# ntampellini/FIRECODE

Hardware: AMD Instinct MI355X
Metric: conformer-pair RMSD alignments/s (higher is better)
Workload: dtype f64

## Files before the change

firecode_amd/csrc/fc_api_ensemble.cpp:

```cpp
#include <algorithm>
#include <cmath>
#include <cstdlib>
#include <memory>

#include "fc_internal.h"

namespace fc {

static int make_selection(const uint8_t *atom_mask, int64_t A_all, std::vector<int32_t> &sel) {
  sel.clear();
  for (int64_t a = 0; a < A_all; ++a)
    if (atom_mask == nullptr || atom_mask[a]) sel.push_back((int32_t)a);
  if (sel.empty()) return set_error(FC_E_INVALID, "atom_mask selects no atom");
  return FC_OK;
}

int ensemble_build_finish(fc_ensemble *e) {
  if (!e->g_max_pending) return FC_OK;
  e->g_max_pending = false;
  FC_TRY(sync());
  std::memcpy(&e->g_max, ctx().pinned_word, sizeof(double));
  auto *gmax_dev = reinterpret_cast<unsigned long long *>(e->counters.p) + (kCounters - 1);
  FC_HIP_TRY(hipMemsetAsync(gmax_dev, 0, sizeof(unsigned long long), ctx().stream));
  return FC_OK;
// ... 283 lines not shown
  FC_REQUIRE(P >= 0, "P < 0");
  if (P == 0) return FC_OK;
  FC_REQUIRE(pair_i && pair_j && rmsd_out && maxdev_out, "NULL pointer argument");
  for (int64_t k = 0; k < P; ++k)
    FC_REQUIRE(pair_i[k] >= 0 && pair_i[k] < ens->N && pair_j[k] >= 0 && pair_j[k] < ens->N,
               "pair %lld = (%lld, %lld) out of range [0, %lld)", (long long)k,
               (long long)pair_i[k], (long long)pair_j[k], (long long)ens->N);
  FC_TRY(ensure_init());
  DevBuf di, dj, dr, dm;
  FC_TRY(upload(di, pair_i, (size_t)P));
  FC_TRY(upload(dj, pair_j, (size_t)P));
  FC_TRY(dr.reserve((size_t)P * sizeof(double)));
  FC_TRY(dm.reserve((size_t)P * sizeof(double)));
  FC_TRY(launch_pairs_exact(ens, di.as<int64_t>(), dj.as<int64_t>(), P, dr.as<double>(),
                            dm.as<double>(), nullptr, inverted));
  FC_TRY(d2h(rmsd_out, dr.p, (size_t)P * sizeof(double)));
  FC_TRY(d2h(maxdev_out, dm.p, (size_t)P * sizeof(double)));
  return sync();
}
int fc_ensemble_rmsd_pairs(fc_ensemble *ens, const int64_t *pair_i, const int64_t *pair_j,
                           int64_t P, double *rmsd_out, double *maxdev_out) {
  return ensemble_rmsd_pairs(ens, pair_i, pair_j, P, rmsd_out, maxdev_out, false);
}
int fc_ensemble_rmsd_pairs_inv(fc_ensemble *ens, const int64_t *pair_i, const int64_t *pair_j, int64_t P, double *rmsd_out,
                               double *maxdev_out) {
  return ensemble_rmsd_pairs(ens, pair_i, pair_j, P, rmsd_out, maxdev_out, true);
}

static int kabsch_rmsd_pairs(const double *coords, int64_t N, int64_t A, const uint8_t *atom_mask, const int64_t *pair_i,
                             const int64_t *pair_j, int64_t P, int center, double *rmsd_out, double *maxdev_out,
                             bool inverted) {
  FC_API_LOCK;
  fc_ensemble *e = nullptr;
  FC_TRY(fc_ensemble_create(coords, N, A, atom_mask, center, &e));
  const int rc = ensemble_rmsd_pairs(e, pair_i, pair_j, P, rmsd_out, maxdev_out, inverted);
  fc_ensemble_destroy(e);
  return rc;
}
int fc_kabsch_rmsd_pairs(const double *coords, int64_t N, int64_t A, const uint8_t *atom_mask,
                         const int64_t *pair_i, const int64_t *pair_j, int64_t P, int center,
                         double *rmsd_out, double *maxdev_out) {
  return kabsch_rmsd_pairs(coords, N, A, atom_mask, pair_i, pair_j, P, center, rmsd_out, maxdev_out, false);
}
int fc_kabsch_rmsd_pairs_inv(const double *coords, int64_t N, int64_t A, const uint8_t *atom_mask, const int64_t *pair_i,
                             const int64_t *pair_j, int64_t P, int center, double *rmsd_out, double *maxdev_out) {
  return kabsch_rmsd_pairs(coords, N, A, atom_mask, pair_i, pair_j, P, center, rmsd_out, maxdev_out, true);
}

static bool rmsd_and_max_tiled(const fc_ensemble *ens) {
  const size_t lds_m = ((size_t)(((ens->A + 3) / 4 + 1) / 2) * 384 + 16 + 128) * sizeof(double) + 1024;
  return lds_m <= kLdsLimit && (uint64_t)((ens->A + 3) / 4 * 4) * 3 * (uint64_t)ens->Npad < (1ull << 32);
}

static int rmsd_and_max_all(fc_ensemble *ens, double *rmsd_out, double *maxdev_out, double *ms_kernel) {
  FC_TRY(ensure_init());
  const int64_t N = ens->N;
  if (N == 0) return FC_OK;
  Context &c = ctx();
  DevBuf dr, dm;
  const size_t bytes = (size_t)N * N * sizeof(double);
  FC_TRY(dr.reserve(bytes));
  FC_TRY(dm.reserve(bytes));
  const bool tiled = rmsd_and_max_tiled(ens);
  unsigned long long cnt[16] = {0};
  if (tiled) {
    FC_TRY(ensemble_shard(ens, 0, 1, 256));
    FC_HIP_TRY(hipMemsetAsync(ens->counters.p, 0, 16 * sizeof(uint64_t), c.stream));
  } else {
    FC_HIP_TRY(hipMemsetAsync(dr.p, 0, bytes, c.stream));
    FC_HIP_TRY(hipMemsetAsync(dm.p, 0, bytes, c.stream));
  }
  FC_HIP_TRY(hipEventRecord(c.ev0, c.stream));
  if (tiled) FC_TRY(launch_rmsd_values(ens, 0.0, dr.as<double>(), dm.as<double>()));
  else FC_TRY(launch_matrix_exact(ens, dr.as<double>(), dm.as<double>()));
  FC_HIP_TRY(hipEventRecord(c.ev1, c.stream));
  if (tiled) FC_TRY(d2h(cnt, ens->counters.p, sizeof cnt));
  FC_TRY(sync());
  FC_TRY(elapsed_ms(c.ev0, c.ev1, ms_kernel));
  if (tiled && cnt[6] > (unsigned long long)ens->pairq_cap) {
    FC_HIP_TRY(hipMemsetAsync(ens->counters.p, 0, 16 * sizeof(uint64_t), c.stream));
    FC_TRY(launch_rmsd_values(ens, 0.0, dr.as<double>(), dm.as<double>(), 0, 1, true));
    FC_TRY(d2h(cnt, ens->counters.p, sizeof cnt));
    FC_TRY(sync());
  }
  if (tiled && cnt[6] > (unsigned long long)ens->pairq_cap) {
    FC_HIP_TRY(hipMemsetAsync(dr.p, 0, bytes, c.stream));
    FC_HIP_TRY(hipMemsetAsync(dm.p, 0, bytes, c.stream));
    FC_TRY(launch_matrix_exact(ens, dr.as<double>(), dm.as<double>()));
  }
  if (rmsd_out) FC_TRY(launch_mirror_upper(dr.as<double>(), N));
  if (maxdev_out) FC_TRY(launch_mirror_upper(dm.as<double>(), N));
  if (rmsd_out) FC_TRY(d2h(rmsd_out, dr.p, bytes));
  if (maxdev_out) FC_TRY(d2h(maxdev_out, dm.p, bytes));
  return sync();
}

static int bench_rmsd_and_max_all(fc_ensemble *ens, int64_t reps, double *ms_kernel_mean, double *ms_total,
                                  int64_t *stats, const int64_t *sample_i = nullptr, const int64_t *sample_j = nullptr,
                                  int64_t P = 0, double *sample_rmsd = nullptr, double *sample_maxdev = nullptr) {
  FC_TRY(ensure_init());
  const int64_t N = ens->N;
  FC_REQUIRE(N >= 2, "needs at least two conformers");
  Context &c = ctx();
  DevBuf dr, dm;
  const size_t bytes = (size_t)N * N * sizeof(double);
  FC_TRY(dr.reserve(bytes));
  FC_TRY(dm.reserve(bytes));
  const bool tiled = rmsd_and_max_tiled(ens);
  const int64_t rank = comm_rank(), world = comm_world();
  FC_REQUIRE(tiled || world == 1, "structures beyond the tiled kernel are not sharded");
  if (tiled) FC_TRY(ensemble_shard(ens, 0, 1, 256));
  FC_TRY(timing_events(2 * reps + 2));
  std::vector<hipEvent_t> &ev = c.ev_pool;
  FC_HIP_TRY(hipEventRecord(ev[2 * reps], c.stream));
  for (int64_t r = 0; r < reps; ++r) {
    if (tiled) {
      FC_HIP_TRY(hipMemsetAsync(ens->counters.p, 0, 16 * sizeof(uint64_t), c.stream));
      FC_HIP_TRY(hipEventRecord(ev[2 * r], c.stream));
      c.mark_after_screen = ev[2 * r + 1];
      const int rc = launch_rmsd_values(ens, 0.0, dr.as<double>(), dm.as<double>(), rank, world);
      c.mark_after_screen = nullptr;
      FC_TRY(rc);
    } else {
      FC_HIP_TRY(hipEventRecord(ev[2 * r], c.stream));
      FC_TRY(launch_matrix_exact(ens, dr.as<double>(), dm.as<double>()));
      FC_HIP_TRY(hipEventRecord(ev[2 * r + 1], c.stream));
    }
  }
  FC_HIP_TRY(hipEventRecord(ev[2 * reps + 1], c.stream));
  unsigned long long cnt[16] = {0};
  if (tiled) FC_TRY(d2h(cnt, ens->counters.p, sizeof cnt));
  FC_TRY(sync());
  double mean = 0.0;
  FC_TRY(mean_elapsed_ms(ev, reps, 2, 1, &mean));
  if (ms_kernel_mean) *ms_kernel_mean = mean;
  FC_TRY(elapsed_ms(ev[2 * reps], ev[2 * reps + 1], ms_total));
  if (stats) {
    stats[0] = owned_pairs(N, 128, rank, world);
    stats[1] = (int64_t)cnt[6];
    stats[2] = tiled ? 1 : 0;
    stats[3] = (int64_t)cnt[kCntGeneralForm];
  }
  if (tiled && cnt[6] > (unsigned long long)ens->pairq_cap)
    return set_error(FC_E_LIMIT, "%llu degenerate pairs exceed the fix-up queue (%lld)", cnt[6], (long long)ens->pairq_cap);
  if (P > 0) {
    DevBuf di, dj, sr, sm;
    FC_TRY(upload(di, sample_i, (size_t)P));
    FC_TRY(upload(dj, sample_j, (size_t)P));
    FC_TRY(sr.reserve((size_t)P * sizeof(double)));
    FC_TRY(sm.reserve((size_t)P * sizeof(double)));
    FC_TRY(launch_gather_matrix_pairs(dr.as<double>(), dm.as<double>(), N, di.as<int64_t>(), dj.as<int64_t>(), P,
                                      sr.as<double>(), sm.as<double>()));
    FC_TRY(d2h(sample_rmsd, sr.p, (size_t)P * sizeof(double)));
    FC_TRY(d2h(sample_maxdev, sm.p, (size_t)P * sizeof(double)));
    FC_TRY(sync());
  }
  return FC_OK;
}

int fc_ensemble_rmsd_matrix(fc_ensemble *ens, double *rmsd_out, double *maxdev_out) {
  FC_API_LOCK;
  FC_REQUIRE(ens && rmsd_out && maxdev_out, "NULL pointer argument");
  return rmsd_and_max_all(ens, rmsd_out, maxdev_out, nullptr);
}
// ... 94 lines not shown
```

firecode_amd/csrc/fc_kabsch.hip:

```cpp
#include <type_traits>

#include "fc_internal.h"
#include <vector>
#include "fc_kabsch_math.h"

#include <algorithm>
#include <cstdlib>

namespace fc {

__global__ void __launch_bounds__(256)
k_prep(const double *__restrict__ coords, int64_t N, int64_t A_all, const int32_t *__restrict__ sel,
       int64_t A, int center, int64_t Npad, double *__restrict__ Xs, double *__restrict__ G,
       double *__restrict__ Xa, unsigned long long *__restrict__ gmax_bits,
       const int32_t *__restrict__ conf_idx) {
  const int64_t n = (int64_t)blockIdx.x * blockDim.x + threadIdx.x;
  if (n >= Npad) return;
  for (int64_t a = A; a < ((A + 3) & ~(int64_t)3); ++a) {
    Xs[(a * 3 + 0) * Npad + n] = 0.0;
    Xs[(a * 3 + 1) * Npad + n] = 0.0;
    Xs[(a * 3 + 2) * Npad + n] = 0.0;
  }
  if (n >= N) {
    for (int64_t a = 0; a < A; ++a) {
// ... 617 lines not shown
  if (i0 >= N) return;
  if (j0 + TC - 1 <= i0) return;
  uint32_t *__restrict__ sq32_wave = reinterpret_cast<uint32_t *>(stageQ) + wv * (kStagePairs * 2 / NW);
  int n_staged32 = 0;
  (void)sq32_wave;
  (void)n_staged32;

  {
    const int n_runs = TC == 64 ? KS * 6 : (TC == 32 ? KS * 3 : ((KS + 1) >> 1) * 3);
    const int cs_l = TC == 64 ? lane >> 4 : lane >> 5, k1_l = TC == 64 ? (lane >> 3) & 1 : (lane >> 3) & 3, c15_l = (lane & 7) * 2;
    for (int q = wv; q < n_runs; q += NW) {
      const int sc = TC == 64 ? q >> 1 : q, kh = TC == 64 ? q & 1 : 0;
      const int sg = sc / 3, c = sc - sg * 3;
      int a = sg * 4 + kh * 2 + k1_l;
      if (TC == 16) {
        a = (sg * 2 + cs_l) * 4 + k1_l;
        a = a < KS * 4 ? a : KS * 4 - 1;
      }
      const double *src = Xs + (int64_t)(a * 3 + c) * Npad + j0 + (TC == 16 ? 0 : cs_l * 16) + c15_l;
      __builtin_amdgcn_global_load_lds((const __attribute__((address_space(1))) void *)src,
                                       (__attribute__((address_space(3))) void *)(lds + q * 128), 16, 0, 0);
    }
    for (int idx = tid; idx < TC + IB; idx += NW * 64) {
      const int64_t g = idx < TC ? j0 + idx : i0 + (idx - TC);
      ldsG[idx] = g < Npad ? G[g] : 0.0;
    }
    if (tid < kStagePairs) stageQ[tid] = ~0ull;
    if (tid < kStageWords) stageW[tid] = ~0u;
    if (tid < 2) stageN[tid] = 0u;
    __syncthreads();
#ifdef FC_TIMELINE
    if (TL && tl && tid == 0) tl[(size_t)b * 4 + 1] = wall_clock64();
#endif
  }
  const int kq = lane >> 4, l15 = lane & 15;
  const int lcol = MODE == 2 ? 4 * (l15 & 3) + (l15 >> 2) : l15;
  const int boff = (kq / KPR) * 128 + (kq % KPR) * 16 + lcol;
  uint16_t *bits16 = reinterpret_cast<uint16_t *>(bits);

  double a0[3], a1[3], a2[3];
  int pre_it = -1;
  int n_general = 0;
  (void)n_general;
  (void)general_only;
  const int tpb = IB >> 4;
  auto tile_row = [&](int it_) -> int64_t {
    if constexpr (MODE == 2) {
      const int k = it_ / tpb;
      return global_block(lb + k, rank, world) * IB + (int64_t)(it_ - k * tpb) * 16;
    } else {
      return i0 + (int64_t)it_ * 16;
    }
  };
  auto row_offsets = [&](int it_, unsigned (&vo)[3]) {
    const int64_t ib_ = tile_row(it_);
#pragma unroll
    for (int c = 0; c < 3; ++c) vo[c] = (unsigned)(((int64_t)(kq * 3 + c) * Npad + ib_ + l15) * 8);
  };
  auto fetch_a_at = [&](double (&a)[3], unsigned (&vo)[3], int sx) {
    const int sl = sx < KS ? sx : KS - 1;
    const char *__restrict__ xs_s = reinterpret_cast<const char *>(Xs + (int64_t)sl * 12 * Npad);
#pragma unroll
    for (int c = 0; c < 3; ++c) {
      asm volatile("" : "+v"(vo[c]));
      a[c] = *reinterpret_cast<const double *>(xs_s + vo[c]);
    }
  };

  for (int it = it_first + wv; it < it_last; it += NW) {
    const int64_t ib = tile_row(it);
    if (ib >= N) break;
    if (j0 + TC - 1 <= ib) break;
    const int64_t lrow0 = lb * IB + (int64_t)it * 16;
    double Gp_row = 0.0;
    if constexpr (MODE == 2) Gp_row = G[ib + l15];
    (void)Gp_row;
    unsigned nz = 0;
    unsigned voff[3];
    row_offsets(it, voff);

#pragma unroll 1
    for (int half = 0; half < NU; ++half) {
      const int cs0 = half * NT;
      if (j0 + (cs0 + NT) * 16 - 1 <= ib) {
        if (!VALUES && lane < 16 && ib + lane < N) {
          bits16[((lrow0 + lane) * W + jt) * 4 + cs0] = 0;
          bits16[((lrow0 + lane) * W + jt) * 4 + cs0 + 1] = 0;
        }
        continue;
      }
      if constexpr (MODE == 2) {
        if (j0 + cs0 * 16 >= N) continue;
      }
      d4_t acc[NT][9];

      const double *__restrict__ lb0 = lds + cs0 * SST + boff;
      double b0[NT][3], b1[NT][3];
      const int KSe = KS;
      auto fetch_a = [&](double (&a)[3], int sx) {
        fetch_a_at(a, voff, sx);
      };
      auto fetch_b = [&](double (&b)[NT][3], int sx) {
        const int sl = sx < KS ? sx : KS - 1;
        const double *__restrict__ lb_s = lb0 + koff(sl);
#pragma unroll
        for (int t = 0; t < NT; ++t)
#pragma unroll
          for (int c = 0; c < 3; ++c) b[t][c] = lb_s[c * CST + t * SST];
      };
      auto mma = [&](const double (&a)[3], const double (&b)[NT][3], auto first_) {
        constexpr bool first = decltype(first_)::value;
#pragma unroll
        for (int x = 0; x < 3; ++x)
#pragma unroll
          for (int y = 0; y < 3; ++y)
#pragma unroll
            for (int t = 0; t < NT; ++t) {
              const d4_t c_in = first ? d4_t{0.0, 0.0, 0.0, 0.0} : acc[t][x * 3 + y];
              acc[t][x * 3 + y] = MODE == 2 ? __builtin_amdgcn_mfma_f64_16x16x4f64(b[t][y], a[x], c_in, 0, 0, 0)
                                            : __builtin_amdgcn_mfma_f64_16x16x4f64(a[x], b[t][y], c_in, 0, 0, 0);
            }
      };
      if (pre_it != it) {
        fetch_a_at(a0, voff, 0);
        fetch_a_at(a1, voff, 1);
        fetch_a_at(a2, voff, 2);
      }
      fetch_b(b0, 0);
      fetch_b(b1, 1);
#define FC_KSTEP(AX, BX, U)             \
  if (sgrp + (U) < KSe) {               \
    mma(AX, BX, std::false_type{});     \
    fetch_a(AX, sgrp + (U) + 3);        \
    fetch_b(BX, sgrp + (U) + 2);        \
  }
      mma(a0, b0, std::true_type{});
      fetch_a(a0, 3);
      fetch_b(b0, 2);
      for (int sgrp = 1; sgrp < KSe; sgrp += 6) {
        FC_KSTEP(a1, b1, 0)
        FC_KSTEP(a2, b0, 1)
        FC_KSTEP(a0, b1, 2)
        FC_KSTEP(a1, b0, 3)
        FC_KSTEP(a2, b1, 4)
        FC_KSTEP(a0, b0, 5)
      }
#undef FC_KSTEP
      {
        const bool same_tile = half < NU - 1 && !(MODE == 2 && j0 + (cs0 + NT) * 16 >= N);
        const int nit = same_tile ? it : it + NW;
        bool more = same_tile;
        if (!same_tile && nit < it_last) {
          const int64_t nib = tile_row(nit);
          more = nib < N && !(j0 + TC - 1 <= nib);
        }
        if (more) {
          unsigned vn[3];
          row_offsets(nit, vn);
          fetch_a_at(a0, vn, 0);
          fetch_a_at(a1, vn, 1);
          fetch_a_at(a2, vn, 2);
          pre_it = nit;
        } else {
          pre_it = -1;
        }
      }
      const int n32 = (int)N, ib32 = (int)ib;
#pragma unroll
      for (int t = 0; t < NT; ++t) {
        const int cs = cs0 + t;
        const int j = (int)j0 + cs * 16 + l15;
        const double Gq = ldsG[cs * 16 + l15];
        uint64_t mr[4] = {0, 0, 0, 0};
        if (MODE == 2) {
          const int i = ib32 + l15;
          const int jb = (int)j0 + cs * 16 + 4 * kq;
          const double Gp = Gp_row;
          double nR[4][9];
          bool ok4[4];
          double msdA4[4] = {0.0, 0.0, 0.0, 0.0};
          {
            if constexpr (COL0) {
              double B4[4][9], GG[4], lam4[4];
#pragma unroll
              for (int r = 0; r < 4; ++r) {
                GG[r] = Gp + ldsG[cs * 16 + 4 * kq + r];
#pragma unroll
                for (int e = 0; e < 9; ++e) B4[r][e] = acc[t][e][r];
              }
              QcpLeanPoly P4[4];
              double dl4[4];
              qcp_lean_eigenvalues4(B4, GG, P4, lam4, dl4);
              bool conv4[4];
#pragma unroll
              for (int r = 0; r < 4; ++r) conv4[r] = qcp_lean_converged(lam4[r], dl4[r]);
              bool all_lean = true, try_col0 = general_only == 0;
              const double k_small = 2e-10 / (double)A;
#pragma unroll
              for (int r = 0; r < 4; ++r) {
                double Qr[4], nqr;
                bool lean = false;
                if (try_col0) {
                  ok4[r] = qcp_lean_quaternion_col0(B4[r], P4[r].n2, lam4[r], conv4[r], Qr, nqr);
                  lean = __builtin_amdgcn_ballot_w64(!(ok4[r] || i >= n32 || jb + r >= n32)) == 0ull;
                  try_col0 = lean;
                }
                if (!lean) ok4[r] = qcp_lean_quaternion_raw(B4[r], P4[r].n2, lam4[r], conv4[r], Qr, nqr);
                all_lean = all_lean && lean;
                if constexpr (EIG) {
                  msdA4[r] = GG[r] - 2.0 * lam4[r];
                  if (!(msdA4[r] > k_small * GG[r] * GG[r])) ok4[r] = false, msdA4[r] = 0.0;
                }
                if (!lean && !ok4[r]) Qr[0] = 1.0, Qr[1] = 0.0, Qr[2] = 0.0, Qr[3] = 0.0, nqr = 1.0;
                neg_rotation_from_raw_quaternion(Qr, nqr, nR[r]);
              }
              if (!all_lean) ++n_general;
            } else {
              double B4[4][9], GG[4], Q44[4][4], nq4[4], lam4[4];
#pragma unroll
              for (int r = 0; r < 4; ++r) {
                GG[r] = Gp + ldsG[cs * 16 + 4 * kq + r];
#pragma unroll
                for (int e = 0; e < 9; ++e) B4[r][e] = acc[t][e][r];
              }
              kabsch_quaternion_qcp_lean4(B4, GG, Q44, nq4, ok4, EIG ? lam4 : nullptr);
              ++n_general;
              if constexpr (EIG) {
                const double k_small = 2e-10 / (double)A;
#pragma unroll
                for (int r = 0; r < 4; ++r) {
                  msdA4[r] = GG[r] - 2.0 * lam4[r];
                  if (!(msdA4[r] > k_small * GG[r] * GG[r])) ok4[r] = false, msdA4[r] = 0.0;
                }
              }
#pragma unroll
              for (int r = 0; r < 4; ++r) {
                if (!ok4[r]) Q44[r][0] = 1.0, Q44[r][1] = 0.0, Q44[r][2] = 0.0, Q44[r][3] = 0.0, nq4[r] = 1.0;
                neg_rotation_from_raw_quaternion(Q44[r], nq4[r], nR[r]);
              }
            }
          }
          typedef double d2_t __attribute__((ext_vector_type(2)));
          const double *__restrict__ qcol = lds + cs * SST + 4 * kq;
          const double *__restrict__ prow_u = Xs + ib;
          const unsigned l15u = (unsigned)l15;
// ... 107 lines not shown
            double PA[3], PB[3];
            load_pq(U0{}, PA, QA);
            for (int g = 0; g < n_groups; ++g) {
              load_pq(U1{}, PB, QB);
              FC_SB;
              accumulate(PA, QA);
              FC_SB;
              load_pq(U2{}, PA, QA);
              FC_SB;
              accumulate(PB, QB);
              FC_SB;
              load_pq(U3{}, PB, QB);
              FC_SB;
              accumulate(PA, QA);
              FC_SB;
              qg = TC == 16 ? qcol + koff(g + 1) : qg + 12 * TC;
              if (g + 1 < n_groups || odd_round) load_pq(U0{}, PA, QA);
              FC_SB;
              accumulate(PB, QB);
              FC_SB;
            }
            if (odd_round) {
              load_pq(U1{}, PB, QB);
              FC_SB;
              accumulate(PA, QA);
              FC_SB;
              accumulate(PB, QB);
            }
          }
#undef FC_SB
          if constexpr (EIG) {
#pragma unroll
            for (int r = 0; r < 4; ++r) ssq[r] = msdA4[r];
          }
          const bool row_in = i < n32;
          double *__restrict__ ro = rmsd_out + (int64_t)i * N + jb;
          double *__restrict__ mo = maxdev_out + (int64_t)i * N + jb;
          const double invA = 1.0 / (double)A;
          if (row_in && jb > i && jb + 3 < n32 && ((((int64_t)i * N) & 1) == 0)) {
            *reinterpret_cast<d2_t *>(ro) = d2_t{fc_sqrt_nonneg(ssq[0] * invA), fc_sqrt_nonneg(ssq[1] * invA)};
            *reinterpret_cast<d2_t *>(ro + 2) = d2_t{fc_sqrt_nonneg(ssq[2] * invA), fc_sqrt_nonneg(ssq[3] * invA)};
            *reinterpret_cast<d2_t *>(mo) = d2_t{fc_sqrt_nonneg(mx[0]), fc_sqrt_nonneg(mx[1])};
            *reinterpret_cast<d2_t *>(mo + 2) = d2_t{fc_sqrt_nonneg(mx[2]), fc_sqrt_nonneg(mx[3])};
          } else {
#pragma unroll
            for (int r = 0; r < 4; ++r) {
              const int j = jb + r;
              if (row_in && j >= i && j < n32) {
                ro[r] = j == i ? 0.0 : fc_sqrt_nonneg(ssq[r] * invA);
                mo[r] = j == i ? 0.0 : fc_sqrt_nonneg(mx[r]);
              }
            }
          }
#pragma unroll
          for (int r = 0; r < 4; ++r) {
            const int j = jb + r;
            const bool redo = row_in && (j > i) && (j < n32) && !ok4[r];
            stage_pairs(__ballot(redo), redo, (unsigned)i, (unsigned)j, stageQ, stageN, pairq, Q, counters, lane);
          }
          continue;
        }
#pragma unroll
        for (int r = 0; r < 4; ++r) {
          const int i = ib32 + kq + 4 * r;
          const double Gp = ldsG[TC + it * 16 + kq + 4 * r];
          double B9[9];
#pragma unroll
          for (int e = 0; e < 9; ++e) B9[e] = acc[t][e][r];
          if (VALUES) {
            double slope;
            const double lam = kabsch_lambda_max(B9, Gp + Gq, &slope);
            const double msdA = (Gp + Gq) - 2.0 * lam;
            const bool in = (j > i) && (j < n32) && (i < n32);
            if (in) rmsd_out[(int64_t)i * N + j] = sqrt(fmax(msdA, 0.0) / (double)A);
            const bool redo = in && (msdA < A_thr2 || !kabsch_lambda_is_sharp(lam, slope, (double)A, msdA));
            stage_pairs(__ballot(redo), redo, (unsigned)i, (unsigned)j, stageQ, stageN, pairq, Q, counters, lane);
            continue;
          }
          bool may = kabsch_may_be_below<ENANT>(B9, Gp + Gq, A_thr2);
          may = may && (j > i) && (j < n32) && (i < n32);
          mr[r] = __ballot(may);
          if constexpr (MODE == 0)
            stage_pairs_wave32<kStagePairs * 2 / NW>(mr[r], may, (unsigned)i, (unsigned)j, (unsigned)i0, (unsigned)j0, sq32_wave,
                                                     n_staged32, pairq, Q, counters, lane);
          else
            stage_pairs(mr[r], may, (unsigned)i, (unsigned)j, stageQ, stageN, pairq, Q, counters, lane);
        }
        if (!VALUES && lane < 16 && ib32 + lane < n32) {
          const int rr = lane >> 2;
          const uint64_t mine = rr == 0 ? mr[0] : rr == 1 ? mr[1] : rr == 2 ? mr[2] : mr[3];
          const unsigned piece = (unsigned)((mine >> (16 * (lane & 3))) & 0xffffull);
          bits16[((lrow0 + lane) * W + jt) * 4 + cs] = (uint16_t)piece;
          nz |= piece;
        }
      }
    }
    if (!VALUES) {
#ifndef FC_ABLATE_PUSH
      const bool has = lane < 16 && nz != 0;
      const uint64_t mw = __ballot(has);
      if (mw != 0) {
        const unsigned n = (unsigned)__popcll(mw);
        const uint32_t word = (uint32_t)((lrow0 + lane) * W + jt);
        unsigned base = 0;
        if (lane == 0) base = atomicAdd(stageN + 1, n);
        base = (unsigned)__builtin_amdgcn_readfirstlane((int)base);
        const unsigned rank_in = (unsigned)__popcll(mw & ((1ull << lane) - 1ull));
        if (base + n <= (unsigned)kStageWords) {
          if (has) stageW[base + rank_in] = word;
        } else {
          unsigned long long gbase = 0;
// ... 1795 lines not shown
    B[6] = fma(pz, qx, B[6]); B[7] = fma(pz, qy, B[7]); B[8] = fma(pz, qz, B[8]);
    g0 += px * px + py * py + pz * pz;
    gn += qx * qx + qy * qy + qz * qz;
  }
  double Q4[4], R[9] = {1.0, 0.0, 0.0, 0.0, 1.0, 0.0, 0.0, 0.0, 1.0};
  if (kabsch_quaternion_qcp(B, g0 + gn, Q4)) rotation_from_quaternion(Q4, R);
  double g = 0.0;
  for (int a = 0; a < A; ++a) {
    const double *__restrict__ row = Xs + (int64_t)a * 3 * Npad;
    double *__restrict__ out = Xf + (int64_t)a * 3 * Npad;
    const double qx = row[n], qy = row[Npad + n], qz = row[2 * Npad + n];
    const double x = R[0] * qx + R[1] * qy + R[2] * qz;
    const double y = R[3] * qx + R[4] * qy + R[5] * qz;
    const double z = R[6] * qx + R[7] * qy + R[8] * qz;
    out[n] = x;
    out[Npad + n] = y;
    out[2 * Npad + n] = z;
    g += x * x + y * y + z * z;
  }
  Gf[n] = g;
}

static int make_frame(fc_ensemble *e, bool with_tiles, bool *made) {
  *made = true;
  if (e->frame_valid && (e->xtf_valid || !with_tiles)) return FC_OK;
  const int64_t n_elems = row_tile_elems(e->Npad, e->A), n_alloc = n_elems + 96;
  if (e->Xf.reserve((size_t)((e->A + 3) / 4 * 4) * 3 * e->Npad * sizeof(double)) != FC_OK ||
      e->Gf.reserve((size_t)e->Npad * sizeof(double)) != FC_OK ||
      (with_tiles && e->Xtf.reserve((size_t)n_alloc * sizeof(double)) != FC_OK)) {
    e->frame_valid = e->xtf_valid = false;
    *made = false;
    return FC_OK;
  }
  if (!e->frame_valid) {
    hipLaunchKernelGGL(k_frame, dim3((unsigned)ceil_div(e->Npad, 64)), dim3(64), 0, ctx().stream, e->Xs.as<double>(), e->N, e->Npad,
                       (int)e->A, e->Xf.as<double>(), e->Gf.as<double>());
    FC_TRY(check_launch("k_frame"));
    e->frame_valid = true;
  }
  if (with_tiles && !e->xtf_valid) {
    hipLaunchKernelGGL(k_row_tiles, dim3((unsigned)ceil_div(n_alloc, 256)), dim3(256), 0, ctx().stream, e->Xf.as<double>(), e->Npad,
                       (int)e->A, n_elems, n_alloc, e->Xtf.as<double>());
    FC_TRY(check_launch("k_row_tiles"));
    e->xtf_valid = true;
  }
  return FC_OK;
}
template <int NW, int TC, bool EIG, bool ROWT, bool COL0 = false>
static int launch_complete_variant(fc_ensemble *e, dim3 grid, size_t lds_m, double A_small, int64_t rb, int64_t rank, int64_t world,
                                   unsigned long long *cnt, const uint64_t *item_table_dev, unsigned long long n_items,
                                   double *rmsd_dev, double *maxdev_dev, uint64_t *timeline_dev, bool frame, bool general_only) {
  const double *xs = frame ? e->Xf.as<double>() : e->Xs.as<double>(), *g = frame ? e->Gf.as<double>() : e->G.as<double>();
  const double *xt = frame ? e->Xtf.as<double>() : e->Xt.as<double>();
  if (lds_m > 64 * 1024) {
    hipError_t err = hipFuncSetAttribute(reinterpret_cast<const void *>(k_simbits_screen_mfma<NW, 2, TC, EIG, false, ROWT, COL0>),
                                         hipFuncAttributeMaxDynamicSharedMemorySize, (int)lds_m);
    if (err != hipSuccess) return set_error(FC_E_HIP, "hipFuncSetAttribute failed: %s", hipGetErrorString(err));
  }
  hipLaunchKernelGGL((k_simbits_screen_mfma<NW, 2, TC, EIG, false, ROWT, COL0>), grid, dim3(NW * 64), lds_m, ctx().stream, xs,
                     g, e->N, e->Npad, (int)e->A, A_small, (int)rb, rank, world, timeline_dev, e->W, nullptr, cnt,
                     e->pairq.as<uint64_t>(), (unsigned long long)e->pairq_cap, item_table_dev, n_items, rmsd_dev, nullptr,
                     maxdev_dev,
                     ROWT ? xt : nullptr, general_only ? 1 : 0);
  return FC_OK;
}

int launch_rmsd_values(fc_ensemble *e, double small_rmsd, double *rmsd_dev, double *maxdev_dev, int64_t rank,
                       int64_t world, bool explicit_sum) {
  const int64_t rb = 128;
  const int64_t n_lblocks = local_block_count(ceil_div(e->N, rb), rank, world);
  if (n_lblocks <= 0) return FC_OK;
  const size_t lds_64 = ((size_t)((e->A + 3) / 4) * 4 * 3 * 64 + 64 + (size_t)rb) * sizeof(double) + kStageBytes;
  const size_t lds_32 = ((size_t)((e->A + 3) / 4) * 4 * 3 * 32 + 32 + (size_t)rb) * sizeof(double) + kStageBytes;
  const size_t lds_16 = ((size_t)(((e->A + 3) / 4 + 1) / 2) * 384 + 16 + (size_t)rb) * sizeof(double) + kStageBytes;
  const bool narrow = lds_64 > kLdsLimit && maxdev_dev != nullptr;
  const int64_t tc = !narrow ? 64 : (lds_32 <= kLdsLimit ? 32 : 16);
  const size_t lds_m = tc == 64 ? lds_64 : (tc == 32 ? lds_32 : lds_16);
  const int64_t NT = e->Npad / tc;
  if (lds_m > kLdsLimit || NT == 0)
    return set_error(FC_E_LIMIT, "A=%lld atoms exceed the LDS column tile of the value kernel", (long long)e->A);
  const bool fits32 = (uint64_t)((e->A + 3) / 4 * 4) * 3 * (uint64_t)e->Npad < (1ull << 32) &&
                      96 * (uint64_t)e->Npad < (1ull << 32);
  if (!fits32) return set_error(FC_E_LIMIT, "ensemble too large for 32-bit operand offsets");
  auto *cnt = reinterpret_cast<unsigned long long *>(e->counters.p);
  const bool two_blocks = 2 * lds_m <= kLdsLimit;
  const bool complete = maxdev_dev != nullptr;
  const void *fn = two_blocks ? reinterpret_cast<const void *>(k_simbits_screen_mfma<4, 1>)
                              : reinterpret_cast<const void *>(k_simbits_screen_mfma<8, 1>);
  if (!complete && lds_m > 64 * 1024) {
    hipError_t err = hipFuncSetAttribute(fn, hipFuncAttributeMaxDynamicSharedMemorySize, (int)lds_m);
    if (err != hipSuccess) return set_error(FC_E_HIP, "hipFuncSetAttribute failed: %s", hipGetErrorString(err));
  }
  const double A_small = (double)e->A * small_rmsd * small_rmsd;
  const int64_t saved_rank = e->rank, saved_world = e->world, saved_rb = e->row_block;
  e->rank = rank; e->world = world; e->row_block = rb;
  int64_t chunk = 0;
  bool tail_order = true;
  if (complete) {
    chunk = two_blocks && !narrow ? kCompleteRowChunk : 1;
    if (const char *v = getenv("FC_COMPLETE_ROW_CHUNK")) chunk = std::min<int64_t>(kItemChunkMax, std::max<int64_t>(1, std::strtoll(v, nullptr, 10)));
    if (const char *v = getenv("FC_COMPLETE_TAIL_ORDER")) tail_order = atoi(v) != 0;
  }
  const int rc_tbl = screen_item_table(e, NT, n_lblocks, true, tc, chunk, tail_order);
  e->rank = saved_rank; e->world = saved_world; e->row_block = saved_rb;
  e->item_key[3] = -1;
  if (rc_tbl != FC_OK) return rc_tbl;
// ... 790 lines not shown
```

firecode_amd/csrc/fc_kabsch_math.h:

```cpp
#pragma once
#include <hip/hip_runtime.h>

namespace fc {

template <int P, int Q>
__host__ __device__ __forceinline__ void jacobi_rot(double (&a)[4][4], double (&v)[4][4], bool late) {
  const double apq = a[P][Q];
  const double g = 100.0 * fabs(apq);
  const double app = a[P][P], aqq = a[Q][Q];
  if (late && (fabs(app) + g == fabs(app)) && (fabs(aqq) + g == fabs(aqq))) {
    a[P][Q] = 0.0;
    a[Q][P] = 0.0;
    return;
  }
  if (apq == 0.0) return;
  const double h = aqq - app;
  double t;
  if (fabs(h) + g == fabs(h)) {
    t = apq / h;
  } else {
    const double theta = 0.5 * h / apq;
    t = 1.0 / (fabs(theta) + sqrt(1.0 + theta * theta));
    if (theta < 0.0) t = -t;
  }
// ... 439 lines not shown
  const double a11 = m00 * L23 - m02 * L03 + m03 * L02;
  const double a12 = -(m00 * L13 - m01 * L03 + m03 * L01);
  const double a13 = m00 * L12 - m01 * L02 + m02 * L01;
  const double a22 = m03 * U13 - m13 * U03 + m33 * U01;
  const double a23 = -(m03 * U12 - m13 * U02 + m23 * U01);
  const double a33 = m02 * U12 - m12 * U02 + m22 * U01;
  double q0 = a00, q1 = a01, q2 = a02, q3 = a03, best = fabs(a00);
  if (fabs(a11) > best) { best = fabs(a11); q0 = a01; q1 = a11; q2 = a12; q3 = a13; }
  if (fabs(a22) > best) { best = fabs(a22); q0 = a02; q1 = a12; q2 = a22; q3 = a23; }
  if (fabs(a33) > best) { best = fabs(a33); q0 = a03; q1 = a13; q2 = a23; q3 = a33; }
  const double scale = fabs(lam) + fabs(Sxx) + fabs(Syy) + fabs(Szz) + fabs(m01) + fabs(m02) + fabs(m03) +
                       fabs(m12) + fabs(m13) + fabs(m23);
  const double nq = q0 * q0 + q1 * q1 + q2 * q2 + q3 * q3;
  if (!(best > 2e-3 * scale * scale * scale) || !(nq > 0.0)) return false;
  const double nrm = fc_rsqrt(nq);
  q0 *= nrm; q1 *= nrm; q2 *= nrm; q3 *= nrm;
  const double r0 = m00 * q0 + m01 * q1 + m02 * q2 + m03 * q3;
  const double r1 = m01 * q0 + m11 * q1 + m12 * q2 + m13 * q3;
  const double r2 = m02 * q0 + m12 * q1 + m22 * q2 + m23 * q3;
  const double r3 = m03 * q0 + m13 * q1 + m23 * q2 + m33 * q3;
  if (!(fmax(fmax(fabs(r0), fabs(r1)), fmax(fabs(r2), fabs(r3))) <= 1e-12 * scale)) return false;
  Q[0] = q0; Q[1] = q1; Q[2] = q2; Q[3] = q3;
  return true;
}

struct QcpLeanPoly {
  double C2, C1, C0, n2;
};
__host__ __device__ __forceinline__ QcpLeanPoly qcp_lean_polynomial(const double (&B)[9]) {
#pragma clang fp contract(fast)
  const double Sxx = B[0], Sxy = B[3], Sxz = B[6];
  const double Syx = B[1], Syy = B[4], Syz = B[7];
  const double Szx = B[2], Szy = B[5], Szz = B[8];
  const double n2 = Sxx * Sxx + Sxy * Sxy + Sxz * Sxz + Syx * Syx + Syy * Syy + Syz * Syz +
                    Szx * Szx + Szy * Szy + Szz * Szz;
  const double c00 = Syy * Szz - Syz * Szy, c01 = Syz * Szx - Syx * Szz, c02 = Syx * Szy - Syy * Szx;
  const double c10 = Sxz * Szy - Sxy * Szz, c11 = Sxx * Szz - Sxz * Szx, c12 = Sxy * Szx - Sxx * Szy;
  const double c20 = Sxy * Syz - Sxz * Syy, c21 = Sxz * Syx - Sxx * Syz, c22 = Sxx * Syy - Sxy * Syx;
  const double detB = Sxx * c00 + Sxy * c01 + Sxz * c02;
  const double e2 = c00 * c00 + c01 * c01 + c02 * c02 + c10 * c10 + c11 * c11 + c12 * c12 +
                    c20 * c20 + c21 * c21 + c22 * c22;
  return QcpLeanPoly{-2.0 * n2, -8.0 * detB, n2 * n2 - 4.0 * e2, n2};
}
__host__ __device__ __forceinline__ bool qcp_lean_step(const QcpLeanPoly &P, double &x, double &delta) {
#pragma clang fp contract(fast)
  const double x2 = x * x;
  const double b = (x2 + P.C2) * x;
  const double a = b + P.C1;
  const double den = 2.0 * x2 * x + b + a;
  delta = (a * x + P.C0) * fc_rcp_approx(den);
  x -= delta;
  return fabs(delta) > 1e-9 * fabs(x);
}
struct QcpAdjCol0 {
  double m01, m02, m03, m11, m12, m13, m22, m23, m33;
  double L01, L02, L03, L12, L13, L23;
  double a00, a01, a02, a03;
};
__host__ __device__ __forceinline__ QcpAdjCol0 qcp_lean_adjugate_col0(const double (&B)[9], double lam) {
#pragma clang fp contract(off)
  const double Sxx = B[0], Sxy = B[3], Sxz = B[6];
  const double Syx = B[1], Syy = B[4], Syz = B[7];
  const double Szx = B[2], Szy = B[5], Szz = B[8];
  QcpAdjCol0 h;
  h.m01 = Syz - Szy, h.m02 = Szx - Sxz, h.m03 = Sxy - Syx;
  h.m11 = (Sxx - Syy - Szz) - lam, h.m12 = Sxy + Syx, h.m13 = Szx + Sxz;
  h.m22 = (-Sxx + Syy - Szz) - lam, h.m23 = Syz + Szy;
  h.m33 = (-Sxx - Syy + Szz) - lam;
  h.L01 = fma(h.m02, h.m13, -(h.m12 * h.m03)), h.L02 = fma(h.m02, h.m23, -(h.m22 * h.m03)), h.L03 = fma(h.m02, h.m33, -(h.m23 * h.m03));
  h.L12 = fma(h.m12, h.m23, -(h.m22 * h.m13)), h.L13 = fma(h.m12, h.m33, -(h.m23 * h.m13)), h.L23 = fma(h.m22, h.m33, -(h.m23 * h.m23));
  h.a00 = fma(h.m13, h.L12, fma(h.m11, h.L23, -(h.m12 * h.L13)));
  h.a01 = -fma(h.m13, h.L02, fma(h.m01, h.L23, -(h.m12 * h.L03)));
  h.a02 = fma(h.m13, h.L01, fma(h.m01, h.L13, -(h.m11 * h.L03)));
  h.a03 = -fma(h.m12, h.L01, fma(h.m01, h.L12, -(h.m11 * h.L02)));
  return h;
}
__host__ __device__ __forceinline__ bool qcp_lean_converged(double lam, double delta) {
  return fabs(delta) <= 1e-9 * fabs(lam);
}
__host__ __device__ __forceinline__ bool qcp_lean_quaternion_raw(const double (&B)[9], double n2, double lam, bool converged,
                                                                 double (&Q)[4], double &nq_out) {
#pragma clang fp contract(fast)
  const double Sxx = B[0], Syy = B[4], Szz = B[8];
  const QcpAdjCol0 h = qcp_lean_adjugate_col0(B, lam);
  const double m00 = (Sxx + Syy + Szz) - lam, m01 = h.m01, m02 = h.m02, m03 = h.m03;
  const double m11 = h.m11, m12 = h.m12, m13 = h.m13, m22 = h.m22, m23 = h.m23, m33 = h.m33;
  const double L01 = h.L01, L02 = h.L02, L03 = h.L03, L12 = h.L12, L13 = h.L13, L23 = h.L23;
  const double U01 = m00 * m11 - m01 * m01, U02 = m00 * m12 - m02 * m01, U03 = m00 * m13 - m03 * m01;
  const double U12 = m01 * m12 - m02 * m11, U13 = m01 * m13 - m03 * m11;
  const double a00 = h.a00, a01 = h.a01, a02 = h.a02, a03 = h.a03;
  const double a11 = m00 * L23 - m02 * L03 + m03 * L02;
  const double a12 = -(m00 * L13 - m01 * L03 + m03 * L01);
  const double a13 = m00 * L12 - m01 * L02 + m02 * L01;
  const double a22 = m03 * U13 - m13 * U03 + m33 * U01;
  const double a23 = -(m03 * U12 - m13 * U02 + m23 * U01);
  const double a33 = m02 * U12 - m12 * U02 + m22 * U01;
  double q0 = a00, q1 = a01, q2 = a02, q3 = a03, best = fabs(a00);
  if (fabs(a11) > best) { best = fabs(a11); q0 = a01; q1 = a11; q2 = a12; q3 = a13; }
  if (fabs(a22) > best) { best = fabs(a22); q0 = a02; q1 = a12; q2 = a22; q3 = a23; }
  if (fabs(a33) > best) { best = fabs(a33); q0 = a03; q1 = a13; q2 = a23; q3 = a33; }
  const double nq = fma(q3, q3, fma(q2, q2, fma(q0, q0, q1 * q1)));
  const bool simple = best * best > (2e-3 * 27.0) * (2e-3 * 27.0) * (n2 * n2) * n2;
  Q[0] = q0; Q[1] = q1; Q[2] = q2; Q[3] = q3;
  nq_out = nq;
  return converged && simple && nq > 0.0;
}
__host__ __device__ __forceinline__ bool qcp_lean_quaternion_raw(const double (&B)[9], const QcpLeanPoly &P, double lam,
                                                                 double delta, double (&Q)[4], double &nq_out) {
  return qcp_lean_quaternion_raw(B, P.n2, lam, qcp_lean_converged(lam, delta), Q, nq_out);
}
__host__ __device__ __forceinline__ bool qcp_lean_quaternion_col0(const double (&B)[9], double n2, double lam, bool converged,
                                                                  double (&Q)[4], double &nq_out) {
#pragma clang fp contract(off)
  const QcpAdjCol0 h = qcp_lean_adjugate_col0(B, lam);
  const double q0 = h.a00, q1 = h.a01, q2 = h.a02, q3 = h.a03, best = fabs(h.a00);
  const double nq = fma(q3, q3, fma(q2, q2, fma(q0, q0, q1 * q1)));
  const bool simple = best * best > (2e-3 * 27.0) * (2e-3 * 27.0) * (n2 * n2) * n2;
  Q[0] = q0; Q[1] = q1; Q[2] = q2; Q[3] = q3;
  nq_out = nq;
  return converged && simple && nq > 0.0 && best * best >= 0.6 * nq;
}
__host__ __device__ __forceinline__ bool qcp_lean_quaternion_col0(const double (&B)[9], const QcpLeanPoly &P, double lam,
                                                                  double delta, double (&Q)[4], double &nq_out) {
  return qcp_lean_quaternion_col0(B, P.n2, lam, qcp_lean_converged(lam, delta), Q, nq_out);
}
__host__ __device__ __forceinline__ bool qcp_lean_quaternion(const double (&B)[9], const QcpLeanPoly &P, double lam,
                                                             double delta, double (&Q)[4]) {
  double nq;
  const bool ok = qcp_lean_quaternion_raw(B, P, lam, delta, Q, nq);
  const double nrm = fc_rsqrt(nq);
  Q[0] *= nrm; Q[1] *= nrm; Q[2] *= nrm; Q[3] *= nrm;
  return ok;
}

__host__ __device__ __forceinline__ bool kabsch_quaternion_qcp_lean(const double (&B)[9], double GpGq, double (&Q)[4],
                                                                    int *iterations = nullptr) {
  const QcpLeanPoly P = qcp_lean_polynomial(B);
  double x = 0.5 * GpGq, delta = 0.0;
  int it = 0;
  for (; it < 64; ++it) {
    const bool moving = qcp_lean_step(P, x, delta);
#if defined(__HIP_DEVICE_COMPILE__)
    if (__builtin_amdgcn_ballot_w64(moving) == 0ull) break;
#else
    if (!moving) break;
#endif
  }
  if (iterations) *iterations = it + 1;
  return qcp_lean_quaternion(B, P, x, delta, Q);
}

__host__ __device__ __forceinline__ void qcp_lean_eigenvalues4(const double (&B)[4][9], const double (&GpGq)[4],
                                                               QcpLeanPoly (&P)[4], double (&x)[4], double (&delta)[4]) {
#pragma unroll
  for (int r = 0; r < 4; ++r) {
    P[r] = qcp_lean_polynomial(B[r]);
    x[r] = 0.5 * GpGq[r];
    delta[r] = 0.0;
  }
  for (int it = 0; it < 64; ++it) {
    bool moving = false;
#pragma unroll
    for (int r = 0; r < 4; ++r) moving |= qcp_lean_step(P[r], x[r], delta[r]);
#if defined(__HIP_DEVICE_COMPILE__)
    if (__builtin_amdgcn_ballot_w64(moving) == 0ull) break;
#else
    if (!moving) break;
#endif
  }
}

__host__ __device__ __forceinline__ void kabsch_quaternion_qcp_lean4(const double (&B)[4][9], const double (&GpGq)[4],
                                                                     double (&Q)[4][4], double (&nq)[4], bool (&ok)[4],
                                                                     double *lam_out = nullptr) {
  QcpLeanPoly P[4];
  double x[4], delta[4];
  qcp_lean_eigenvalues4(B, GpGq, P, x, delta);
#pragma unroll
  for (int r = 0; r < 4; ++r) ok[r] = qcp_lean_quaternion_raw(B[r], P[r], x[r], delta[r], Q[r], nq[r]);
  if (lam_out != nullptr) {
#pragma unroll
    for (int r = 0; r < 4; ++r) lam_out[r] = x[r];
  }
}

__host__ __device__ __forceinline__ void rotation_from_quaternion(const double (&Q)[4], double (&R)[9]) {
#pragma clang fp contract(fast)
  const double q0 = Q[0], q1 = Q[1], q2 = Q[2], q3 = Q[3];
  R[0] = q0 * q0 + q1 * q1 - q2 * q2 - q3 * q3;
  R[1] = 2.0 * (q1 * q2 - q0 * q3);
  R[2] = 2.0 * (q1 * q3 + q0 * q2);
  R[3] = 2.0 * (q1 * q2 + q0 * q3);
  R[4] = q0 * q0 - q1 * q1 + q2 * q2 - q3 * q3;
  R[5] = 2.0 * (q2 * q3 - q0 * q1);
  R[6] = 2.0 * (q1 * q3 - q0 * q2);
  R[7] = 2.0 * (q2 * q3 + q0 * q1);
  R[8] = q0 * q0 - q1 * q1 - q2 * q2 + q3 * q3;
}

__host__ __device__ __forceinline__ void neg_rotation_from_quaternion(const double (&Q)[4], double (&R)[9]) {
#pragma clang fp contract(fast)
  const double q0 = Q[0], q1 = Q[1], q2 = Q[2], q3 = Q[3];
  R[0] = q2 * q2 + q3 * q3 - q0 * q0 - q1 * q1;
  R[1] = -2.0 * (q1 * q2 - q0 * q3);
  R[2] = -2.0 * (q1 * q3 + q0 * q2);
  R[3] = -2.0 * (q1 * q2 + q0 * q3);
  R[4] = q1 * q1 + q3 * q3 - q0 * q0 - q2 * q2;
  R[5] = -2.0 * (q2 * q3 - q0 * q1);
  R[6] = -2.0 * (q1 * q3 - q0 * q2);
  R[7] = -2.0 * (q2 * q3 + q0 * q1);
  R[8] = q1 * q1 + q2 * q2 - q0 * q0 - q3 * q3;
}

__host__ __device__ __forceinline__ void neg_rotation_from_raw_quaternion(const double (&Q)[4], double nq, double (&R)[9]) {
#pragma clang fp contract(fast)
  const double q0 = Q[0], q1 = Q[1], q2 = Q[2], q3 = Q[3];
  double inv = fc_rcp_approx(nq);
  inv = fma(fma(-nq, inv, 1.0), inv, inv);
  inv = fma(fma(-nq, inv, 1.0), inv, inv);
  const double t = inv + inv;
  const double p11 = q1 * q1, p22 = q2 * q2;
  R[0] = fma(t, fma(q3, q3, p22), -1.0);
// ... 13 lines not shown
```

firecode_amd/csrc/fc_tuning.h:

```cpp
#pragma once

#if !defined(FC_TUNING_BUILD) &&                                                                                             \
    (defined(FC_TIMELINE) || defined(FC_H2_TIMELINE) || defined(FC_RB_TIMELINE) || defined(FC_TFD_STAMPS) || defined(FC_TFD_STAMPS_SMALL) || defined(FC_H2_ABLATE_K) ||   \
     defined(FC_H2_ABLATE_ROWS) || defined(FC_H2_ABLATE_POLY) || defined(FC_F32_ABLATE_K) || defined(FC_F32_ABLATE_POLY) ||  \
     defined(FC_ABLATE_PUSH) || defined(FC_ABLATE_STAGE) || defined(FC_ABLATE_OVERFLOW) || defined(FC_ABLATE_REDO) ||         \
     defined(FC_RB_NOSTAGE) || defined(FC_RB_NOPASS1) || defined(FC_RB_NOPASS2) || defined(FC_RB_NOJACOBI) ||                \
     defined(FC_RB_NOCOMPUTE) || defined(FC_RB_ROWS_FROM_LDS) || defined(FC_RB_SAMEROW) || defined(FC_RB_WPS) ||              \
     defined(FC_RB_AHEAD) || defined(FC_RB_CHUNK) || defined(FC_H2_WGS) || defined(FC_F32_WGS) || defined(FC_REFINE_ROUNDS) || defined(FC_STAGE_PAIRS_F32) || defined(FC_TS_WGS) || defined(FC_TS_TURN) || defined(FC_KNN_SYM_ROWS) || defined(FC_SUM_SYM_ROWS))
#error "a tuning switch (FC_*TIMELINE / FC_*ABLATE* / FC_RB_* / FC_TFD_STAMPS ...) without -DFC_TUNING_BUILD: see fc_tuning.h"
#endif

#ifdef __cplusplus
namespace fc {
constexpr int64_t kDiverseLanes8MaxN = 10000;
constexpr int kKnnWorkgroupsPerCu = 4;
constexpr int kKnnMaxStrips = 64;
constexpr int kButinaRounds = 16;
constexpr long long kButinaLiveEdges = 1ll << 22;
}
#endif
```

Measured before the change: 21.26 billion.

## Walk row-tile indices incrementally, unroll leading QCP Newton steps, skip idle redo staging

In MODE 2, each wave now steps its row-tile position forward with a running counter instead of recomputing global_block per iteration. It also reuses the current offsets when prefetching within the same tile. The 4-wide QCP eigenvalue solve now uses a reformulated Newton step with an approximate reciprocal, and runs the first iterations unconditionally so no ballot checks them. Redo staging is skipped when no lane in the wave needs it. Risks: the approximate reciprocal may change convergence or accuracy, and a new guard rejects row blocks smaller than NW tiles. Debug-only poison fills and an ablation switch are also added.

```diff
diff --git a/firecode_amd/csrc/fc_api_ensemble.cpp b/firecode_amd/csrc/fc_api_ensemble.cpp
--- a/firecode_amd/csrc/fc_api_ensemble.cpp
+++ b/firecode_amd/csrc/fc_api_ensemble.cpp
@@ -359,6 +359,14 @@
   return lds_m <= kLdsLimit && (uint64_t)((ens->A + 3) / 4 * 4) * 3 * (uint64_t)ens->Npad < (1ull << 32);
 }
 
+static int complete_poison(void *rmsd_dev, void *maxdev_dev, size_t bytes) {
+  const char *v = getenv("FC_COMPLETE_POISON");
+  if (v == nullptr || atoi(v) == 0) return FC_OK;
+  FC_HIP_TRY(hipMemsetAsync(rmsd_dev, 0xff, bytes, ctx().stream));
+  FC_HIP_TRY(hipMemsetAsync(maxdev_dev, 0xff, bytes, ctx().stream));
+  return FC_OK;
+}
+
 static int rmsd_and_max_all(fc_ensemble *ens, double *rmsd_out, double *maxdev_out, double *ms_kernel) {
   FC_TRY(ensure_init());
   const int64_t N = ens->N;
@@ -373,6 +381,7 @@
   if (tiled) {
     FC_TRY(ensemble_shard(ens, 0, 1, 256));
     FC_HIP_TRY(hipMemsetAsync(ens->counters.p, 0, 16 * sizeof(uint64_t), c.stream));
+    FC_TRY(complete_poison(dr.p, dm.p, bytes));
   } else {
     FC_HIP_TRY(hipMemsetAsync(dr.p, 0, bytes, c.stream));
     FC_HIP_TRY(hipMemsetAsync(dm.p, 0, bytes, c.stream));
@@ -417,6 +426,7 @@
   const int64_t rank = comm_rank(), world = comm_world();
   FC_REQUIRE(tiled || world == 1, "structures beyond the tiled kernel are not sharded");
   if (tiled) FC_TRY(ensemble_shard(ens, 0, 1, 256));
+  if (tiled) FC_TRY(complete_poison(dr.p, dm.p, bytes));
   FC_TRY(timing_events(2 * reps + 2));
   std::vector<hipEvent_t> &ev = c.ev_pool;
   FC_HIP_TRY(hipEventRecord(ev[2 * reps], c.stream));
diff --git a/firecode_amd/csrc/fc_kabsch.hip b/firecode_amd/csrc/fc_kabsch.hip
--- a/firecode_amd/csrc/fc_kabsch.hip
+++ b/firecode_amd/csrc/fc_kabsch.hip
@@ -693,11 +693,29 @@
       return i0 + (int64_t)it_ * 16;
     }
   };
-  auto row_offsets = [&](int it_, unsigned (&vo)[3]) {
-    const int64_t ib_ = tile_row(it_);
+  auto row_offsets_at = [&](int64_t ib_, unsigned (&vo)[3]) {
 #pragma unroll
     for (int c = 0; c < 3; ++c) vo[c] = (unsigned)(((int64_t)(kq * 3 + c) * Npad + ib_ + l15) * 8);
   };
+  auto row_offsets = [&](int it_, unsigned (&vo)[3]) { row_offsets_at(tile_row(it_), vo); };
+  int w_k = 0, w_t = 0;
+  int64_t w_row = i0;
+  auto walk_on = [&](int &k_, int &t_, int64_t &row_) {
+    if constexpr (MODE == 2) {
+      t_ += NW;
+      if (t_ >= tpb) {
+        t_ -= tpb;
+        ++k_;
+        row_ = global_block(lb + k_, rank, world) * IB;
+      }
+    }
+  };
+  if constexpr (MODE == 2) {
+    const int it0 = it_first + wv;
+    w_k = it0 / tpb;
+    w_t = it0 - w_k * tpb;
+    w_row = global_block(lb + w_k, rank, world) * IB;
+  }
   auto fetch_a_at = [&](double (&a)[3], unsigned (&vo)[3], int sx) {
     const int sl = sx < KS ? sx : KS - 1;
     const char *__restrict__ xs_s = reinterpret_cast<const char *>(Xs + (int64_t)sl * 12 * Npad);
@@ -708,8 +726,8 @@
     }
   };
 
-  for (int it = it_first + wv; it < it_last; it += NW) {
-    const int64_t ib = tile_row(it);
+  for (int it = it_first + wv; it < it_last; it += NW, walk_on(w_k, w_t, w_row)) {
+    const int64_t ib = MODE == 2 ? w_row + (int64_t)w_t * 16 : tile_row(it);
     if (ib >= N) break;
     if (j0 + TC - 1 <= ib) break;
     const int64_t lrow0 = lb * IB + (int64_t)it * 16;
@@ -718,7 +736,7 @@
     (void)Gp_row;
     unsigned nz = 0;
     unsigned voff[3];
-    row_offsets(it, voff);
+    row_offsets_at(ib, voff);
 
 #pragma unroll 1
     for (int half = 0; half < NU; ++half) {
@@ -791,13 +809,38 @@
         const bool same_tile = half < NU - 1 && !(MODE == 2 && j0 + (cs0 + NT) * 16 >= N);
         const int nit = same_tile ? it : it + NW;
         bool more = same_tile;
+        int64_t nib = ib;
         if (!same_tile && nit < it_last) {
-          const int64_t nib = tile_row(nit);
+#ifdef FC_ABLATE_PREDICT
+          nib = ib;
+#else
+          if constexpr (MODE == 2) {
+            int n_k = w_k, n_t = w_t;
+            int64_t n_row = w_row;
+            walk_on(n_k, n_t, n_row);
+            nib = n_row + (int64_t)n_t * 16;
+          } else {
+            nib = tile_row(nit);
+          }
+#endif
           more = nib < N && !(j0 + TC - 1 <= nib);
         }
         if (more) {
           unsigned vn[3];
-          row_offsets(nit, vn);
+#ifdef FC_ABLATE_PREDICT
+          for (int c = 0; c < 3; ++c) vn[c] = voff[c];
+#else
+          if constexpr (MODE == 2) {
+            if (same_tile) {
+#pragma unroll
+              for (int c = 0; c < 3; ++c) vn[c] = voff[c];
+            } else {
+              row_offsets_at(nib, vn);
+            }
+          } else {
+            row_offsets(nit, vn);
+          }
+#endif
           fetch_a_at(a0, vn, 0);
           fetch_a_at(a1, vn, 1);
           fetch_a_at(a2, vn, 2);
@@ -831,7 +874,7 @@
               }
               QcpLeanPoly P4[4];
               double dl4[4];
-              qcp_lean_eigenvalues4(B4, GG, P4, lam4, dl4);
+              qcp_lean_eigenvalues4_lead(B4, GG, P4, lam4, dl4, 3);
               bool conv4[4];
 #pragma unroll
               for (int r = 0; r < 4; ++r) conv4[r] = qcp_lean_converged(lam4[r], dl4[r]);
@@ -1045,11 +1088,17 @@
               }
             }
           }
+          bool redo4[4], redo_any = false;
 #pragma unroll
           for (int r = 0; r < 4; ++r) {
             const int j = jb + r;
-            const bool redo = row_in && (j > i) && (j < n32) && !ok4[r];
-            stage_pairs(__ballot(redo), redo, (unsigned)i, (unsigned)j, stageQ, stageN, pairq, Q, counters, lane);
+            redo4[r] = row_in && (j > i) && (j < n32) && !ok4[r];
+            redo_any = redo_any || redo4[r];
+          }
+          if (__ballot(redo_any) != 0ull) {
+#pragma unroll
+            for (int r = 0; r < 4; ++r)
+              stage_pairs(__ballot(redo4[r]), redo4[r], (unsigned)i, (unsigned)(jb + r), stageQ, stageN, pairq, Q, counters, lane);
           }
           continue;
         }
@@ -2951,6 +3000,7 @@
                                    double *rmsd_dev, double *maxdev_dev, uint64_t *timeline_dev, bool frame, bool general_only) {
   const double *xs = frame ? e->Xf.as<double>() : e->Xs.as<double>(), *g = frame ? e->Gf.as<double>() : e->G.as<double>();
   const double *xt = frame ? e->Xtf.as<double>() : e->Xt.as<double>();
+  if ((int64_t)NW * 16 > rb) return set_error(FC_E_INTERNAL, "row blocks of %lld rows hold fewer than %d row tiles", (long long)rb, NW);
   if (lds_m > 64 * 1024) {
     hipError_t err = hipFuncSetAttribute(reinterpret_cast<const void *>(k_simbits_screen_mfma<NW, 2, TC, EIG, false, ROWT, COL0>),
                                          hipFuncAttributeMaxDynamicSharedMemorySize, (int)lds_m);
diff --git a/firecode_amd/csrc/fc_kabsch_math.h b/firecode_amd/csrc/fc_kabsch_math.h
--- a/firecode_amd/csrc/fc_kabsch_math.h
+++ b/firecode_amd/csrc/fc_kabsch_math.h
@@ -515,6 +515,19 @@
   x -= delta;
   return fabs(delta) > 1e-9 * fabs(x);
 }
+__host__ __device__ __forceinline__ bool qcp_lean_step_said(const QcpLeanPoly &P, double &x, double &delta) {
+#pragma clang fp contract(off)
+  const double x2 = x * x;
+  const double t = fma(x, x, P.C2);
+  const double b = x * t;
+  const double a = fma(x, t, P.C1);
+  const double den = fma(x, x2 + x2, b) + a;
+  const double rc = fc_rcp_approx(den);
+  const double num = fma(x, a, P.C0);
+  delta = num * rc;
+  x = fma(-num, rc, x);
+  return fabs(delta) > 1e-9 * fabs(x);
+}
 struct QcpAdjCol0 {
   double m01, m02, m03, m11, m12, m13, m22, m23, m33;
   double L01, L02, L03, L12, L13, L23;
@@ -613,24 +626,34 @@
   return qcp_lean_quaternion(B, P, x, delta, Q);
 }
 
-__host__ __device__ __forceinline__ void qcp_lean_eigenvalues4(const double (&B)[4][9], const double (&GpGq)[4],
-                                                               QcpLeanPoly (&P)[4], double (&x)[4], double (&delta)[4]) {
+__host__ __device__ __forceinline__ void qcp_lean_eigenvalues4_lead(const double (&B)[4][9], const double (&GpGq)[4],
+                                                                    QcpLeanPoly (&P)[4], double (&x)[4], double (&delta)[4],
+                                                                    const int n_lead) {
 #pragma unroll
   for (int r = 0; r < 4; ++r) {
     P[r] = qcp_lean_polynomial(B[r]);
     x[r] = 0.5 * GpGq[r];
     delta[r] = 0.0;
   }
-  for (int it = 0; it < 64; ++it) {
+#pragma unroll
+  for (int it = 1; it < n_lead; ++it) {
+#pragma unroll
+    for (int r = 0; r < 4; ++r) (void)qcp_lean_step_said(P[r], x[r], delta[r]);
+  }
+  for (int it = n_lead - 1; it < 64; ++it) {
     bool moving = false;
 #pragma unroll
-    for (int r = 0; r < 4; ++r) moving |= qcp_lean_step(P[r], x[r], delta[r]);
+    for (int r = 0; r < 4; ++r) moving |= qcp_lean_step_said(P[r], x[r], delta[r]);
 #if defined(__HIP_DEVICE_COMPILE__)
     if (__builtin_amdgcn_ballot_w64(moving) == 0ull) break;
 #else
     if (!moving) break;
 #endif
   }
+}
+__host__ __device__ __forceinline__ void qcp_lean_eigenvalues4(const double (&B)[4][9], const double (&GpGq)[4],
+                                                               QcpLeanPoly (&P)[4], double (&x)[4], double (&delta)[4]) {
+  qcp_lean_eigenvalues4_lead(B, GpGq, P, x, delta, 1);
 }
 
 __host__ __device__ __forceinline__ void kabsch_quaternion_qcp_lean4(const double (&B)[4][9], const double (&GpGq)[4],
diff --git a/firecode_amd/csrc/fc_tuning.h b/firecode_amd/csrc/fc_tuning.h
--- a/firecode_amd/csrc/fc_tuning.h
+++ b/firecode_amd/csrc/fc_tuning.h
@@ -3,7 +3,7 @@
 #if !defined(FC_TUNING_BUILD) &&                                                                                             \
     (defined(FC_TIMELINE) || defined(FC_H2_TIMELINE) || defined(FC_RB_TIMELINE) || defined(FC_TFD_STAMPS) || defined(FC_TFD_STAMPS_SMALL) || defined(FC_H2_ABLATE_K) ||   \
      defined(FC_H2_ABLATE_ROWS) || defined(FC_H2_ABLATE_POLY) || defined(FC_F32_ABLATE_K) || defined(FC_F32_ABLATE_POLY) ||  \
-     defined(FC_ABLATE_PUSH) || defined(FC_ABLATE_STAGE) || defined(FC_ABLATE_OVERFLOW) || defined(FC_ABLATE_REDO) ||         \
+     defined(FC_ABLATE_PUSH) || defined(FC_ABLATE_STAGE) || defined(FC_ABLATE_OVERFLOW) || defined(FC_ABLATE_REDO) || defined(FC_ABLATE_PREDICT) || \
      defined(FC_RB_NOSTAGE) || defined(FC_RB_NOPASS1) || defined(FC_RB_NOPASS2) || defined(FC_RB_NOJACOBI) ||                \
      defined(FC_RB_NOCOMPUTE) || defined(FC_RB_ROWS_FROM_LDS) || defined(FC_RB_SAMEROW) || defined(FC_RB_WPS) ||              \
      defined(FC_RB_AHEAD) || defined(FC_RB_CHUNK) || defined(FC_H2_WGS) || defined(FC_F32_WGS) || defined(FC_REFINE_ROUNDS) || defined(FC_STAGE_PAIRS_F32) || defined(FC_TS_WGS) || defined(FC_TS_TURN) || defined(FC_KNN_SYM_ROWS) || defined(FC_SUM_SYM_ROWS))
```

Measured after the change: 21.41 billion, median of 6. About the same (+0.7%).
